# lukehinds/fastllm

Hardware: NVIDIA B200
Metric: decode_tokens_per_s (higher is better)
Workload: dtype bf16

## Files before the change

### fastllm_b200/csrc/decode_persistent.cuh

```cuda
#pragma once
#include "attn_decode.cuh"
#include "common.cuh"
#include "dense_ops.cuh"
#include "gemm_tc.cuh"
#include "gemv.cuh"
#include "mma.cuh"

namespace fl {

constexpr int kPkConsumerWarps = 8;
constexpr int kPkConsumers = kPkConsumerWarps * 32;
constexpr int kPkThreads = kPkConsumers + 32;
constexpr int kPkBlockRows = 16;
constexpr int kPkChunkCols = 1024;
constexpr int kPkStageBytes = kPkBlockRows * kPkChunkCols * 2;
constexpr int kPkMaxStages = 6;
constexpr int kPkMaxSlots = 96;
constexpr int kPkMaxNormK = 8192;

struct PkLayer {
    const uint16_t* wqkv;
    const float* bqkv;
    const uint16_t* wo;
    const uint16_t* wgu;
    const uint16_t* wdown;
    const float* ln1;
    const float* ln2;
};

struct PkArgs {
    const PkLayer* layers;
    int L;
    const uint16_t* embed;
    const uint16_t* lm_head;
    const float* final_norm;
    int H, I, V, nh, nkv, d, nqkv, max_pos;
    float eps, qscale;
    const float* rope_cos;
    const float* rope_sin;
    uint16_t* kpool;
    uint16_t* vpool;
    size_t layer_pool_elems;
    const int* page_table;
    StepState* state;
    float* resid;
    float* q;
    float* attn_out;
    uint16_t* xhl;
    float* act;
    float* logits;
    float* part_acc;
    float* part_ml;
    int* counters;
    int nsplit;
    float* amax_val;
    int* amax_idx;
    uint32_t* ids;
    uint32_t* next_ids;
    uint32_t* trace;
    int* trace_pos;
    unsigned int* gbar;
    int nsteps, feedback;
    int nstages;
    int xs_floats;
    int kcap;
    const CUtensorMap* tmaps;
    unsigned int* pool;
    int partial_rows;
    int tp, rank;
    float* peer_part[8];
    unsigned int* peer_flag[8];
    float* peer_amax[8];
    float* peer_logits[8];
    unsigned int ar_epoch0;
    int* comm_err;
    long long* dbg;
};

struct PkSplit {
    int s0, s1;
    int pool0, npool;
    int ncc;
};
constexpr int kPkStaticNum = 30;
constexpr int kPkPoolCap = 8;

__device__ __forceinline__ PkSplit pk_split(int N, int K, int cta, int ncta, bool dynamic) {
    PkSplit p;
    const int nblk = N / kPkBlockRows;
    p.ncc = (K + kPkChunkCols - 1) / kPkChunkCols;
    if (dynamic) {
        const int S = (int)((long long)nblk * kPkStaticNum / 32) / ncta;
        p.s0 = cta * S; p.s1 = p.s0 + S;
        p.pool0 = ncta * S; p.npool = nblk - p.pool0;
    } else {
        p.s0 = (int)((long long)nblk * cta / ncta); p.s1 = (int)((long long)nblk * (cta + 1) / ncta);
        p.pool0 = nblk; p.npool = 0;
    }
    return p;
}

constexpr int kPkMetaEnd = 1 << 30;

__device__ __forceinline__ void pk_named_sync() { asm volatile("bar.sync 1, %0;" ::"n"(kPkConsumers) : "memory"); }

__device__ __forceinline__ unsigned int ld_acquire_gpu(const unsigned int* p) {
    unsigned int v;
    asm volatile("ld.acquire.gpu.global.u32 %0, [%1];" : "=r"(v) : "l"(p) : "memory");
    return v;
}

__device__ __forceinline__ uint4 ldcg_u4(const void* p) {
    uint4 r;
    asm volatile("ld.global.cg.v4.u32 {%0, %1, %2, %3}, [%4];" : "=r"(r.x), "=r"(r.y), "=r"(r.z), "=r"(r.w) : "l"(p));
    return r;
}
// ... 8 lines not shown
    const PkLayer& lw = a.layers[g >> 2];
    switch (g & 3) {
        case 0: W = lw.wqkv; N = a.nqkv; K = a.H; break;
        case 1: W = lw.wo; N = a.H; K = a.nh * a.d; break;
        case 2: W = lw.wgu; N = 2 * a.I; K = a.H; break;
        default: W = lw.wdown; N = a.H; K = a.I; break;
    }
}

__device__ __forceinline__ void pk_grid_barrier(unsigned int* ctr, unsigned int& epoch, int tid) {
    pk_named_sync();
    epoch += 1;
    if (tid == 0) {
        asm volatile("red.release.gpu.global.add.u32 [%0], %1;" ::"l"(ctr), "r"(1u) : "memory");
        const unsigned int target = epoch * gridDim.x;
        while (ld_acquire_gpu(ctr) < target) { }
    }
    pk_named_sync();
}

__device__ __forceinline__ void st_release_sys(unsigned int* p, unsigned int v) {
    asm volatile("st.release.sys.global.u32 [%0], %1;" ::"l"(p), "r"(v) : "memory");
}
__device__ __forceinline__ unsigned int ld_acquire_sys(const unsigned int* p) {
    unsigned int v;
    asm volatile("ld.acquire.sys.global.u32 %0, [%1];" : "=r"(v) : "l"(p) : "memory");
    return v;
}
__device__ __forceinline__ void pk_wait_flag(const unsigned int* flag, unsigned int epoch, int* err) {
    const long long t0 = clock64();
    while ((int)(ld_acquire_sys(flag) - epoch) < 0) {
        if (clock64() - t0 > 4000000000LL) {
            *err = 1;
            break;
        }
    }
}

template <int D>
__global__ void __launch_bounds__(kPkThreads, 1) decode_persistent_kernel(const PkArgs a) {
    extern __shared__ __align__(1024) uint8_t smem[];
    uint8_t* ring = smem;
    float* xs = reinterpret_cast<float*>(smem + (size_t)a.nstages * kPkStageBytes);
    float* partial = xs + a.xs_floats;
    float* sc = partial + (size_t)a.partial_rows * kPkConsumerWarps;
    float* red = sc + kAttnMaxRep * kKvPage;
    float* alpha_s = red + 32;
    float* mrun = alpha_s + 8;
    float* lrun = mrun + 8;
    int* s_flag = reinterpret_cast<int*>(lrun + 8);
    __shared__ __align__(8) uint64_t full[kPkMaxStages];
    __shared__ __align__(8) uint64_t empty[kPkMaxStages];
    __shared__ __align__(8) uint64_t xbar;
    __shared__ int2 meta[kPkMaxStages];
    __shared__ int blk_rows[kPkMaxSlots];

    const int tid = threadIdx.x, lane = tid & 31, warp = tid >> 5;
    const int cta = blockIdx.x, ncta = gridDim.x;
    const int NS = a.nstages;
    const int nq = a.nh * a.d;

    if (tid == 0) {
        for (int s = 0; s < NS; ++s) {
            mbar_init(&full[s], 1);
            mbar_init(&empty[s], kPkConsumerWarps);
        }
        mbar_init(&xbar, 1);
        mbar_fence_init();
    }
    __syncthreads();

    if (warp == kPkConsumerWarps) {
        if (lane != 0) return;
        unsigned int c = 0;
        const uint64_t pol_first = l2_policy_evict_first();
        const bool dynamic = a.tp == 1 && a.pool != nullptr;
        for (int step = 0; step < a.nsteps; ++step) {
            for (int g = 0; g <= 4 * a.L; ++g) {
                const uint16_t* W;
                int N, K;
                pk_phase(a, g, W, N, K);
                const PkSplit sp = pk_split(N, K, cta, ncta, dynamic);
                const bool pdbg = a.dbg != nullptr && cta == 0 && g < 4 * a.L && (g >> 2) == a.L / 2;
                int pn = 0;
                auto fetch_block = [&](int blk) {
                    for (int cc = 0; cc < sp.ncc; ++cc) {
                        const int st = c % NS;
                        mbar_wait(&empty[st], ((c / NS) & 1) ^ 1);
                        ++c;
                        meta[st] = make_int2(blk * kPkBlockRows, cc | (cc == sp.ncc - 1 ? 1 << 16 : 0));
                        if (pdbg) {
                            long long t;
                            asm volatile("mov.u64 %0, %%globaltimer;" : "=l"(t));
                            if (pn < 8) a.dbg[660 + (g & 3) * 10 + pn] = t;
                            a.dbg[660 + (g & 3) * 10 + 8] = t;
                            a.dbg[660 + (g & 3) * 10 + 9] = ++pn;
                        }
                        mbar_expect_tx(&full[st], kPkStageBytes);
                        asm volatile(
                            "cp.async.bulk.tensor.3d.shared::cluster.global.mbarrier::complete_tx::bytes.L2::cache_hint [%0], [%1, {%2, %3, %4}], [%5], %6;" ::"r"(
                                smem_u32(ring + (size_t)st * kPkStageBytes)),
                            "l"(a.tmaps + g), "r"(0), "r"(blk * kPkBlockRows), "r"(cc * (kPkChunkCols / 64)), "r"(smem_u32(&full[st])), "l"(pol_first)
                            : "memory");
                    }
                };
                for (int blk = sp.s0; blk < sp.s1; ++blk) fetch_block(blk);
                for (int taken = 0; sp.npool > 0 && taken < kPkPoolCap; ++taken) {
                    const int t = (int)atomicAdd(a.pool + g, 1u);
                    if (t >= sp.npool) break;
                    fetch_block(sp.pool0 + t);
                }
                const int st = c % NS;
                mbar_wait(&empty[st], ((c / NS) & 1) ^ 1);
                meta[st] = make_int2(0, kPkMetaEnd);
                mbar_arrive(&full[st]);
                ++c;
            }
        }
        return;
    }
// ... 149 lines not shown
                    v[j] = make_float4(bf16lo(e.x), bf16hi(e.x), bf16lo(e.y), bf16hi(e.y));
                    if (resid_out) reinterpret_cast<float4*>(resid_out)[i] = v[j];
                } else {
                    v[j] = __ldcg(reinterpret_cast<const float4*>(src) + i);
                }
            }
        }
#pragma unroll
        for (int j = 0; j < NV; ++j) {
            ss = fmaf(v[j].x, v[j].x, ss); ss = fmaf(v[j].y, v[j].y, ss); ss = fmaf(v[j].z, v[j].z, ss); ss = fmaf(v[j].w, v[j].w, ss);
        }
        const float tot = block_sum(ss);
        const float m = sqrtf(tot / (float)K + a.eps);
#pragma unroll
        for (int j = 0; j < NV; ++j) {
            const int i = tid + j * kPkConsumers;
            const float4 x = v[j];
            if (i < K / 4) store_x4(i, make_float4(x.x / m * wv[j].x, x.y / m * wv[j].y, x.z / m * wv[j].z, x.w / m * wv[j].w));
        }
        zero_x_tail(K);
        pk_named_sync();
    };
    unsigned int xphase = 0;
    auto load_x_plain = [&](const uint16_t* hi, int K) {
        if (tid == 0) {
            asm volatile("fence.proxy.async;" ::: "memory");
            mbar_expect_tx(&xbar, (uint32_t)K * 4u);
            bulk_g2s(xh, hi, (uint32_t)K * 2u, &xbar);
            bulk_g2s(xl, hi + K, (uint32_t)K * 2u, &xbar);
        }
        zero_x_tail(K);
        mbar_wait(&xbar, xphase & 1u);
        xphase ^= 1u;
        pk_named_sync();
    };

    auto prefetch_vec = [&](const float* p, int n) {
        for (int i = tid * 32; i < n; i += kPkConsumers * 32) asm volatile("prefetch.global.L2 [%0];" ::"l"(p + i));
    };
    int dbg_i = 0;
    auto stamp = [&](int l) {
        if (a.dbg != nullptr && cta == 0 && tid == 0 && l == a.L / 2) {
            long long t;
            asm volatile("mov.u64 %0, %%globaltimer;" : "=l"(t));
            a.dbg[dbg_i] = t;
        }
        ++dbg_i;
    };
    const int n_rep = a.nh / a.nkv;
    constexpr int LPT = D / 8, TPW = 32 / LPT;
    const int grp = lane / LPT, gl = lane % LPT;
    int item0 = cta;
    asm volatile("" : "+r"(item0));

    for (int step = 0; step < a.nsteps; ++step) {
        const uint32_t tok_id = __ldcg(a.ids);
        const int rope_pos = min(__ldcg(&a.state->rope_pos), a.max_pos - 1);
        const int kv_base = __ldcg(&a.state->kv_base[0]);
        const int slot = kv_base;
        const int len = kv_base + 1;
        const int page_of_slot = __ldg(a.page_table + slot / kKvPage);

        for (int l = 0; l < a.L; ++l) {
            const PkLayer& lw = a.layers[l];
            uint16_t* kpool = a.kpool + (size_t)l * a.layer_pool_elems;
            uint16_t* vpool = a.vpool + (size_t)l * a.layer_pool_elems;

            prefetch_vec(lw.ln2, a.H);
            dbg_i = 0;
            dbg_layer = l;
            stamp(l);
            if (l == 0) {
                const int npages = (len + kKvPage - 1) / kKvPage;
                for (int i = tid * 32; i < npages; i += kPkConsumers * 32) asm volatile("prefetch.global.L1 [%0];" ::"l"(a.page_table + i));
            }
            if (l == 0)
                load_x_rmsnorm(nullptr, true, a.embed + (size_t)tok_id * a.H, lw.ln1, a.H, cta == 0 ? a.resid : nullptr);
            else
                load_x_rmsnorm(a.resid, false, nullptr, lw.ln1, a.H, nullptr);
            stamp(l);
            {
                const int nslots = consume(a.H);
                stamp(l);
                const int d = a.d, half = d >> 1;
                for (int e = tid; e < nslots * (kPkBlockRows / 2); e += kPkConsumers) {
                    const int ra = grow(2 * e);
                    float va = row_sum(2 * e), vb = row_sum(2 * e + 1);
                    if (lw.bqkv) { va += lw.bqkv[ra]; vb += lw.bqkv[ra + 1]; }
                    const int hh = ra / d, j = (ra % d) >> 1;
                    if (hh < a.nh + a.nkv) {
                        const float cs = a.rope_cos[(size_t)rope_pos * half + j], sn = a.rope_sin[(size_t)rope_pos * half + j];
                        const float o1 = va * cs - vb * sn, o2 = va * sn + vb * cs;
                        if (hh < a.nh) {
                            a.q[(size_t)hh * d + j] = o1;
                            a.q[(size_t)hh * d + j + half] = o2;
                        } else {
                            uint16_t* kp = kpool + (((size_t)page_of_slot * a.nkv + (hh - a.nh)) * kKvPage + slot % kKvPage) * d;
                            kp[j] = f32_to_bf16_rne(o1);
                            kp[j + half] = f32_to_bf16_rne(o2);
                        }
                    } else {
                        uint16_t* vp = vpool + (((size_t)page_of_slot * a.nkv + (hh - a.nh - a.nkv)) * kKvPage + slot % kKvPage) * d;
                        *reinterpret_cast<uint32_t*>(vp + 2 * j) = (uint32_t)f32_to_bf16_rne(va) | ((uint32_t)f32_to_bf16_rne(vb) << 16);
                    }
                }
            }
            stamp(l);
            pk_grid_barrier(a.gbar, epoch, tid);
            if (cta == 0 && tid == 0 && a.pool != nullptr) atomicExch(a.pool + (4 * l), 0u);
            stamp(l);

            {
                constexpr int HG = 4;
                constexpr int NG = kPkConsumerWarps * TPW;
                constexpr int BATCH = 4;
                const int npages = (len + kKvPage - 1) / kKvPage;
                const int per = (npages + a.nsplit - 1) / a.nsplit;
                float* gacc = xs;
                float* gml = xs + NG * HG * D;
                for (int item = item0; item < a.nkv * a.nsplit; item += ncta) {
                    const int kvh = item / a.nsplit, split = item % a.nsplit;
                    const int tok0 = split * per * kKvPage, tok1 = min(min((split + 1) * per, npages) * kKvPage, len);
                    const int gidx = warp * TPW + grp;
                    for (int h0 = 0; h0 < n_rep; h0 += HG) {
                        float qv[HG][8], acc[HG][8], mr[HG], lr[HG];
#pragma unroll
                        for (int h = 0; h < HG; ++h) {
                            mr[h] = -INFINITY;
                            lr[h] = 0.f;
#pragma unroll
                            for (int i = 0; i < 8; ++i) acc[h][i] = 0.f;
                            if (h0 + h < n_rep) {
                                const float4* qp = reinterpret_cast<const float4*>(a.q + (size_t)(kvh * n_rep + h0 + h) * D + gl * 8);
                                const float4 q0 = __ldcg(qp), q1 = __ldcg(qp + 1);
                                qv[h][0] = q0.x * a.qscale; qv[h][1] = q0.y * a.qscale; qv[h][2] = q0.z * a.qscale; qv[h][3] = q0.w * a.qscale;
                                qv[h][4] = q1.x * a.qscale; qv[h][5] = q1.y * a.qscale; qv[h][6] = q1.z * a.qscale; qv[h][7] = q1.w * a.qscale;
                            } else {
#pragma unroll
                                for (int i = 0; i < 8; ++i) qv[h][i] = 0.f;
                            }
                        }
                        for (int tb0 = tok0; tb0 < tok1; tb0 += NG * BATCH) {
                            const int tb = tb0 + gidx;
                            uint4 kw[BATCH], vw[BATCH];
#pragma unroll
                            for (int it = 0; it < BATCH; ++it) {
                                const int tk = tb + it * NG;
                                if (tk < tok1) {
                                    const size_t base = (((size_t)__ldg(a.page_table + tk / kKvPage) * a.nkv + kvh) * kKvPage + tk % kKvPage) * D + gl * 8;
                                    kw[it] = ldcg_u4(kpool + base);
                                    vw[it] = ldcg_u4(vpool + base);
                                } else {
                                    kw[it] = make_uint4(0u, 0u, 0u, 0u);
                                    vw[it] = kw[it];
                                }
                            }
#pragma unroll
                            for (int it = 0; it < BATCH; ++it) {
                                const bool valid = tb + it * NG < tok1;
                                const float kf[8] = {bf16lo(kw[it].x), bf16hi(kw[it].x), bf16lo(kw[it].y), bf16hi(kw[it].y),
                                                     bf16lo(kw[it].z), bf16hi(kw[it].z), bf16lo(kw[it].w), bf16hi(kw[it].w)};
                                const float vf[8] = {bf16lo(vw[it].x), bf16hi(vw[it].x), bf16lo(vw[it].y), bf16hi(vw[it].y),
                                                     bf16lo(vw[it].z), bf16hi(vw[it].z), bf16lo(vw[it].w), bf16hi(vw[it].w)};
#pragma unroll
                                for (int h = 0; h < HG; ++h) {
                                    float sv = kf[0] * qv[h][0];
#pragma unroll
                                    for (int i = 1; i < 8; ++i) sv = fmaf(kf[i], qv[h][i], sv);
#pragma unroll
                                    for (int o = LPT / 2; o > 0; o >>= 1) sv += __shfl_xor_sync(0xFFFFFFFFu, sv, o);
                                    if (valid) {
                                        const float m_new = fmaxf(mr[h], sv);
                                        const float al = expf(mr[h] - m_new), pr = expf(sv - m_new);
                                        lr[h] = lr[h] * al + pr;
                                        mr[h] = m_new;
#pragma unroll
                                        for (int i = 0; i < 8; ++i) acc[h][i] = fmaf(acc[h][i], al, pr * vf[i]);
                                    }
                                }
                            }
                        }
#pragma unroll
                        for (int h = 0; h < HG; ++h) {
                            float* dst = gacc + ((size_t)gidx * HG + h) * D + gl * 8;
#pragma unroll
                            for (int i = 0; i < 8; ++i) dst[i] = acc[h][i];
                            if (gl == 0) {
                                gml[(gidx * HG + h) * 2] = mr[h];
                                gml[(gidx * HG + h) * 2 + 1] = lr[h];
                            }
                        }
                        pk_named_sync();
                        for (int i = tid; i < HG * D; i += kPkConsumers) {
                            const int h = i / D, dd = i % D;
                            if (h0 + h < n_rep) {
                                float M = -INFINITY;
#pragma unroll
                                for (int g = 0; g < NG; ++g) M = fmaxf(M, gml[(g * HG + h) * 2]);
                                float num = 0.f, den = 0.f;
                                if (M != -INFINITY) {
#pragma unroll
                                    for (int g = 0; g < NG; ++g) {
                                        const float wg = expf(gml[(g * HG + h) * 2] - M);
                                        num = fmaf(wg, gacc[((size_t)g * HG + h) * D + dd], num);
                                        den = fmaf(wg, gml[(g * HG + h) * 2 + 1], den);
                                    }
                                }
                                const size_t pidx = (size_t)(kvh * n_rep + h0 + h) * a.nsplit + split;
                                a.part_acc[pidx * D + dd] = num;
                                if (dd == 0) {
                                    a.part_ml[pidx * 2] = M;
                                    a.part_ml[pidx * 2 + 1] = den;
                                }
                            }
                        }
                        pk_named_sync();
                    }
                    __threadfence();
                    pk_named_sync();
                    if (tid == 0) *s_flag = (atomicAdd(&a.counters[kvh], 1) == a.nsplit - 1);
                    pk_named_sync();
                    if (*s_flag) {
                        __threadfence();
                        float* cm = xs;
                        float* cden = cm + kAttnMaxRep * a.nsplit;
                        if (warp < n_rep) {
                            const int h = warp;
                            const size_t base = (size_t)(kvh * n_rep + h) * a.nsplit;
                            float mstar = -INFINITY;
                            for (int s = lane; s < a.nsplit; s += 32) mstar = fmaxf(mstar, __ldcg(a.part_ml + (base + s) * 2));
                            mstar = warp_max(mstar);
                            float den = 0.f;
                            for (int s = lane; s < a.nsplit; s += 32) {
                                const float ms = __ldcg(a.part_ml + (base + s) * 2);
                                const float w = (ms == -INFINITY) ? 0.f : expf(ms - mstar);
                                cm[h * a.nsplit + s] = w;
                                den = fmaf(w, __ldcg(a.part_ml + (base + s) * 2 + 1), den);
                            }
                            den = warp_sum(den);
                            if (lane == 0) cden[h] = den;
                        }
                        pk_named_sync();
                        constexpr int D4 = D / 4;
                        for (int i = tid; i < n_rep * D4; i += kPkConsumers) {
                            const int h = i / D4, c4 = i % D4;
                            const float4* src = reinterpret_cast<const float4*>(a.part_acc + (size_t)(kvh * n_rep + h) * a.nsplit * D) + c4;
                            float4 num = make_float4(0.f, 0.f, 0.f, 0.f);
#pragma unroll 8
                            for (int s = 0; s < a.nsplit; ++s) {
                                const float w = cm[h * a.nsplit + s];
                                if (w != 0.f) {
                                    const float4 v = __ldcg(src + (size_t)s * D4);
                                    num.x = fmaf(w, v.x, num.x); num.y = fmaf(w, v.y, num.y); num.z = fmaf(w, v.z, num.z); num.w = fmaf(w, v.w, num.w);
                                }
                            }
                            const float den = cden[h];
                            uint32_t h0, l0, h1, l1;
                            split2(num.x / den, num.y / den, h0, l0);
                            split2(num.z / den, num.w / den, h1, l1);
                            const size_t oi = (size_t)(kvh * n_rep + h) * D + c4 * 4;
                            *reinterpret_cast<uint2*>(a.xhl + oi) = make_uint2(h0, h1);
                            *reinterpret_cast<uint2*>(a.xhl + nq + oi) = make_uint2(l0, l1);
                        }
                        if (tid == 0) a.counters[kvh] = 0;
                    }
                    pk_named_sync();
                }
            }
            stamp(l);
            pk_grid_barrier(a.gbar, epoch, tid);
            stamp(l);

            prefetch_vec(l + 1 < a.L ? a.layers[l + 1].ln1 : a.final_norm, a.H);
            load_x_plain(a.xhl, nq);
            stamp(l);
            {
                const int nslots = consume(nq);
                stamp(l);
                if (a.tp > 1) {
                    allreduce_resid_add(nslots);
                } else {
                    for (int e = tid; e < nslots * (kPkBlockRows / 2); e += kPkConsumers) {
                        float2* p = reinterpret_cast<float2*>(a.resid + grow(2 * e));
                        float2 v = __ldcg(p);
                        v.x += row_sum(2 * e);
                        v.y += row_sum(2 * e + 1);
                        *p = v;
                    }
                }
            }
            stamp(l);
            pk_grid_barrier(a.gbar, epoch, tid);
            if (cta == 0 && tid == 0 && a.pool != nullptr) atomicExch(a.pool + (4 * l + 1), 0u);
            stamp(l);

            load_x_rmsnorm(a.resid, false, nullptr, lw.ln2, a.H, nullptr);
            stamp(l);
            {
                long long t0c = 0;
                if (a.dbg != nullptr && tid == 0 && l == a.L / 2) asm volatile("mov.u64 %0, %%globaltimer;" : "=l"(t0c));
                const int nslots = consume(a.H);
                if (a.dbg != nullptr && tid == 0 && l == a.L / 2) {
                    long long t1c;
                    unsigned int smid;
                    asm volatile("mov.u64 %0, %%globaltimer;" : "=l"(t1c));
                    asm volatile("mov.u32 %0, %%smid;" : "=r"(smid));
                    a.dbg[64 + cta * 4] = t0c; a.dbg[64 + cta * 4 + 1] = t1c; a.dbg[64 + cta * 4 + 2] = smid; a.dbg[64 + cta * 4 + 3] = nslots;
                }
                stamp(l);
                for (int e = tid; e < nslots * (kPkBlockRows / 2); e += kPkConsumers) {
                    const float g = row_sum(2 * e), u = row_sum(2 * e + 1);
                    const float av = g / (1.f + expf(-g)) * u;
                    uint16_t ah, al;
                    split_hi_lo(av, ah, al);
                    const int aj = grow(2 * e) >> 1;
                    a.xhl[2 * nq + aj] = ah;
                    a.xhl[2 * nq + a.I + aj] = al;
                }
            }
// ... 122 lines not shown
```

### fastllm_b200/csrc/fl_lib.cu

```cuda
#include <cmath>
#include <sstream>
#include <thread>

#include "attn_decode.cuh"
#include "attn_mma.cuh"
#include "comm.cuh"
#include "decode_persistent.cuh"
#include "dense_ops.cuh"
#include "gemm_tc.cuh"
#include "elementwise.cuh"
#include "gemv.cuh"
#include "model.cuh"
#include "sampler.hpp"
#include "synth.cuh"

namespace fl {

thread_local std::string g_last_error;
std::atomic<uint64_t> g_launches{0};
Profiler g_prof;
NcclApi g_nccl;
PeerComm g_peer;
static std::atomic<int> g_device{-1};

// ... 487 lines not shown
            tm.push_back(make_tmap_pk(w.layers[l].wdown, w.H, w.I));
        }
        tm.push_back(make_tmap_pk(w.lm_head, w.V, w.H));
        w.pk_tmaps.alloc(tm.size());
        FL_CUDA(cudaMemcpy(w.pk_tmaps.p, tm.data(), tm.size() * sizeof(CUtensorMap), cudaMemcpyHostToDevice));
    }
    w.finalized = true;
}

static void tp_allreduce_sum(LaunchCtx& lc, float* buf, size_t count) {
    FL_CHECK(g_nccl.comm != nullptr, FL_ERR_STATE, "tensor parallelism: fl_comm_init has not been called");
    g_nccl.check(g_nccl.AllReduce(buf, buf, count, ncclFloat32, ncclSum, g_nccl.comm, lc.stream), "ncclAllReduce");
    count_launch(lc);
}
static void tp_allgather(LaunchCtx& lc, const float* send, float* recv, size_t count) {
    FL_CHECK(g_nccl.comm != nullptr, FL_ERR_STATE, "tensor parallelism: fl_comm_init has not been called");
    g_nccl.check(g_nccl.AllGather(send, recv, count, ncclFloat32, g_nccl.comm, lc.stream), "ncclAllGather");
    count_launch(lc);
}
struct A2aSeg {
    const void* send;
    void* recv;
    size_t bytes;
    bool replicate;
};
static void ep_alltoall(LaunchCtx& lc, const A2aSeg* segs, int nseg) {
    FL_CHECK(g_nccl.comm != nullptr, FL_ERR_STATE, "expert parallelism: fl_comm_init has not been called");
    g_nccl.check(g_nccl.GroupStart(), "ncclGroupStart");
    for (int i = 0; i < nseg; ++i) {
        const A2aSeg& sg = segs[i];
        for (int p = 0; p < g_nccl.world; ++p) {
            const uint8_t* sp = (const uint8_t*)sg.send + (sg.replicate ? 0 : (size_t)p * sg.bytes);
            g_nccl.check(g_nccl.Send(sp, sg.bytes, ncclUint8, p, g_nccl.comm, lc.stream), "ncclSend");
            g_nccl.check(g_nccl.Recv((uint8_t*)sg.recv + (size_t)p * sg.bytes, sg.bytes, ncclUint8, p, g_nccl.comm, lc.stream), "ncclRecv");
        }
    }
    g_nccl.check(g_nccl.GroupEnd(), "ncclGroupEnd");
    count_launch(lc);
}

constexpr int kPassRows = 2;

static void plan_persistent(fl_cache& c) {
    const Weights& w = *c.w;
    PkPlan& p = c.pk;
    p.ok = false;
    if (env_flag("FL_NO_PERSISTENT")) return;
    if (w.tp > 1 && (!g_peer.ready || w.H > PeerComm::kMaxH || (size_t)w.Vfull > PeerComm::kMaxVocab || w.tp > PeerComm::kMaxTp)) return;
    if (w.cfg.arch == FL_ARCH_MIXTRAL) return;
    const int nq = w.nh * w.d;
    if (!(w.d == 64 || w.d == 128)) return;
    if (w.H < 2048 || nq < 256 || w.I < 256) return;
    if (w.pk_tmaps.p == nullptr || w.nqkv % 16 || w.H % 16 || (2 * w.I) % 16 || w.V % 16 || w.H > kPkMaxNormK) return;
    int kmax = (std::max(w.H, std::max(nq, w.I)) + kPkChunkCols - 1) / kPkChunkCols * kPkChunkCols;
    p.xs_floats = (int)align_up((size_t)std::max(std::max(kmax + 16, 8192 + 512), 8 * kNumSMs + 16), 4);
    int slots = 0;
    for (int N : {w.nqkv, w.H, 2 * w.I, w.V}) {
        const int nblk = N / kPkBlockRows;
        slots = std::max(slots, w.tp == 1 ? nblk / kNumSMs + kPkPoolCap : (nblk + kNumSMs - 1) / kNumSMs + 1);
    }
    if (slots > kPkMaxSlots) return;
    p.partial_rows = slots * kPkBlockRows;
    const size_t fixed = (size_t)p.xs_floats * 4 + (size_t)p.partial_rows * kPkConsumerWarps * 4 + (size_t)kAttnMaxRep * kKvPage * 4 + 64 * 4;
    const size_t avail = 232448 - 2048;
    if (fixed + 2 * (size_t)kPkStageBytes > avail) return;
    p.nstages = (int)std::min<size_t>(kPkMaxStages, (avail - fixed) / kPkStageBytes);
    p.smem = (size_t)p.nstages * kPkStageBytes + fixed;
    p.nsplit = std::max(1, std::min(c.pages_per_seq, kNumSMs / w.nkv));
    if (p.nsplit > c.nsplit) p.nsplit = c.nsplit;
    int coop = 0;
    FL_CUDA(cudaDeviceGetAttribute(&coop, cudaDevAttrCooperativeLaunch, w.device));
    if (!coop) return;
    c.gbar.alloc(1, true);
    p.ok = true;
}

static void launch_persistent(fl_cache& c, int nsteps, bool feedback) {
    const Weights& w = *c.w;
    PkArgs a{};
    a.layers = w.pk_layers.p; a.L = w.L; a.embed = w.embed; a.lm_head = w.lm_head; a.final_norm = w.final_norm;
    a.H = w.H; a.I = w.I; a.V = w.V; a.nh = w.nh; a.nkv = w.nkv; a.d = w.d; a.nqkv = w.nqkv; a.max_pos = w.max_pos;
    a.eps = w.cfg.norm_eps; a.qscale = (float)(1.0 / std::sqrt((double)w.d));
    a.rope_cos = w.rope_cos; a.rope_sin = w.rope_sin;
    a.kpool = c.kpool.p; a.vpool = c.vpool.p; a.layer_pool_elems = c.layer_pool_elems; a.page_table = c.page_table.p;
    a.state = c.state.p; a.resid = c.resid.p; a.q = c.q.p; a.attn_out = c.attn_out.p; a.act = c.act.p; a.logits = c.logits.p;
    a.part_acc = c.part_acc.p; a.part_ml = c.part_ml.p; a.counters = c.counters.p; a.nsplit = c.pk.nsplit;
    a.amax_val = c.amax_val.p; a.amax_idx = c.amax_idx.p; a.ids = c.ids.p; a.next_ids = c.next_ids.p;
    a.trace = feedback ? c.trace.p : nullptr; a.trace_pos = c.trace_pos.p; a.gbar = c.gbar.p;
    a.nsteps = nsteps; a.feedback = feedback ? 1 : 0; a.nstages = c.pk.nstages; a.xs_floats = c.pk.xs_floats;
    a.partial_rows = c.pk.partial_rows;
    if (c.pk_xhl.p == nullptr) c.pk_xhl.alloc(2 * ((size_t)w.nh * w.d + w.I) + 64, true);
    a.xhl = c.pk_xhl.p;
    a.kcap = (std::max(w.H, std::max(w.nh * w.d, w.I)) + kPkChunkCols - 1) / kPkChunkCols * kPkChunkCols;
    a.tmaps = w.pk_tmaps.p;
    if (c.pk_pool.p == nullptr) c.pk_pool.alloc(4 * (size_t)w.L + 1, true);
    a.pool = c.pk_pool.p;
    a.tp = w.tp; a.rank = w.rank;
    if (w.tp > 1) {
        for (int r = 0; r < w.tp; ++r) {
            uint8_t* base = (uint8_t*)g_peer.peer[r];
            a.peer_part[r] = (float*)(base + PeerComm::kPartOff);
            a.peer_flag[r] = (unsigned int*)(base + PeerComm::kFlagOff);
            a.peer_amax[r] = (float*)(base + PeerComm::kAmaxOff);
            a.peer_logits[r] = (float*)(base + PeerComm::kLogitsOff);
        }
        a.comm_err = (int*)((uint8_t*)g_peer.local + PeerComm::kErrOff);
        a.ar_epoch0 = g_peer.ar_epoch;
        g_peer.ar_epoch += (unsigned int)nsteps * (2u * (unsigned int)w.L + 1u);
    }
    static long long* dbg_buf = nullptr;
    const bool dbg = env_flag("FL_PK_DEBUG");
    if (dbg && !dbg_buf) {
        FL_CUDA(cudaMalloc(&dbg_buf, (64 + 4 * kNumSMs + 64) * sizeof(long long)));
        FL_CUDA(cudaMemset(dbg_buf, 0, (64 + 4 * kNumSMs + 64) * sizeof(long long)));
    }
    a.dbg = dbg ? dbg_buf : nullptr;
    FL_CUDA(cudaMemsetAsync(c.gbar.p, 0, sizeof(unsigned int), c.stream));
    FL_CUDA(cudaMemsetAsync(c.pk_pool.p, 0, (4 * (size_t)w.L + 1) * sizeof(unsigned int), c.stream));
    LaunchCtx lc{c.stream, false};
    lc.cooperative = true;
    const uint64_t bytes = (uint64_t)nsteps * (w.streamed_bytes + (uint64_t)c.kv_len * w.L * w.nkv * w.d * 2 * 2);
    with_head_dim(w.d, [&](auto D) {
        if constexpr (D == 64 || D == 128)
            launch(lc, "decode_persistent", bytes, decode_persistent_kernel<D>, dim3(kNumSMs), dim3(kPkThreads), c.pk.smem, a);
    });
    if (w.tp > 1)
        FL_CUDA(cudaMemcpyAsync(c.logits.p, (uint8_t*)g_peer.local + PeerComm::kLogitsOff, (size_t)w.Vfull * 4, cudaMemcpyDeviceToDevice, c.stream));
    if (dbg) {
        static const char* names[] = {"P1 x(rmsnorm)", "P1 consume qkv", "P1 epilogue", "P1 grid barrier", "P2 attention", "P2 grid barrier",
                                      "P3 x", "P3 consume o", "P3 epilogue", "P3 grid barrier", "P4 x(rmsnorm)", "P4 consume gate/up",
                                      "P4 epilogue", "P4 grid barrier", "P5 x", "P5 consume down", "P5 epilogue", "P5 grid barrier"};
        long long h[40];
        FL_CUDA(cudaStreamSynchronize(c.stream));
        FL_CUDA(cudaMemcpy(h, dbg_buf, sizeof(h), cudaMemcpyDeviceToHost));
        fprintf(stderr, "[FL_PK_DEBUG] warp 0 of CTA 0, clocks waiting for weights / chunks per phase: qkv %lld/%lld o %lld/%lld gateup %lld/%lld down %lld/%lld\n",
                h[32] / 1000, h[32] % 1000, h[33] / 1000, h[33] % 1000, h[34] / 1000, h[34] % 1000, h[35] / 1000, h[35] % 1000);
        fprintf(stderr, "[FL_PK_DEBUG] layer %d, CTA 0 phase times (us):", w.L / 2);
        for (int i = 0; i < 18; ++i) fprintf(stderr, " %s=%.2f;", names[i], (h[i + 1] - h[i]) / 1000.0);
        fprintf(stderr, " layer total=%.2f\n", (h[18] - h[0]) / 1000.0);
        {
            long long pr[40];
            FL_CUDA(cudaMemcpy(pr, dbg_buf + 660, sizeof(pr), cudaMemcpyDeviceToHost));
// ... 1174 lines not shown
```

### fastllm_b200/csrc/model.cuh

```cuda
#pragma once
#include <map>
#include <memory>
#include <set>
#include <string>
#include <vector>

#include "../../include/fastllm_b200.h"
#include "bert_model.cuh"
#include "decode_persistent.cuh"
#include "gemv.cuh"
#include "runtime.cuh"

namespace fl {

struct LayerW {
    uint16_t* wqkv = nullptr;
    float* bqkv = nullptr;
    uint16_t* wo = nullptr;
    uint16_t* wgu = nullptr;
    uint16_t* wdown = nullptr;
    float* ln1 = nullptr;
    float* ln2 = nullptr;
    CUtensorMap tm_wqkv, tm_wo, tm_wgu, tm_wdown;
    float* wgate = nullptr;
    std::vector<uint16_t*> ewgu, ewdown;
    std::vector<CUtensorMap> tm_ewgu, tm_ewdown;
    CUtensorMap tm_ewgu_all, tm_ewdown_all;
};

struct Weights {
    fl_config cfg{};
    int H = 0, I = 0, V = 0, L = 0, nh = 0, nkv = 0, d = 0, max_pos = 0;
    int nqkv = 0;
    int tp = 1, rank = 0;
    int q_head0 = 0, q_real = 0, kv_head0 = 0;
    int E = 0, top_k = 0;
    int ep = 1, E_local = 0;
    bool ep_dp = false;
    int Vfull = 0;
    int device = 0;
    DevBuf<uint8_t> slab;
    uint16_t* embed = nullptr;
    uint16_t* lm_head = nullptr;
    float* final_norm = nullptr;
    std::vector<LayerW> layers;
    DevBuf<PkLayer> pk_layers;
    DevBuf<CUtensorMap> pk_tmaps;
    float* rope_cos = nullptr;
    float* rope_sin = nullptr;
    std::set<std::string> have;
    bool lm_head_loaded = false;
    bool finalized = false;
    uint64_t streamed_bytes = 0;
    CUtensorMap tm_head;
    bool dense_ok = false;
    std::mutex mu;
};

struct PkPlan {
    bool ok = false;
    int nstages = 0, xs_floats = 0, partial_rows = 0, nsplit = 1;
    size_t smem = 0;
};

struct DenseWs {
    size_t rows = 0;
    DevBuf<uint16_t> xhi, xlo;
    DevBuf<float> y;
    DevBuf<float> resid, q;
    DevBuf<float> tp_buf;
    DevBuf<uint16_t> xhi2, xlo2;
    DevBuf<uint16_t> vt;
    size_t vt_pages_cap = 0;
    CUtensorMap tm_vt{};
    DevBuf<float> sk_acc, sk_ml;
    DevBuf<float> moe_out, route_w;
    DevBuf<int> route_sel;
    DevBuf<float> route_margin;
    int route_rows = 0;
    DevBuf<uint16_t> gx_hi, gx_lo;
    DevBuf<int> grp_cnt, grp_pos;
    DevBuf<uint16_t> g_xhi, g_xlo;
    DevBuf<float> g_route;
    DevBuf<float> comb;
    DevBuf<int> counters;
};

struct GraphKey {
    int b;
    int loop;
    bool operator<(const GraphKey& o) const { return b != o.b ? b < o.b : loop < o.loop; }
};
struct GraphEntry {
    cudaGraphExec_t exec = nullptr;
    uint64_t kernels = 0;
};

}

struct fl_model {
    std::shared_ptr<fl::Weights> w;
    std::shared_ptr<fl::BertModel> bert;
};

struct fl_cache {
    std::shared_ptr<fl::Weights> w;
    cudaStream_t stream = nullptr;
    int max_batch = 0, max_seq = 0, pages_per_seq = 0, nsplit = 1;
    int kv_len = 0;
    bool slots_used = false;
    std::vector<int> slot_len;
    fl::DevBuf<int> slot_tab;
    fl::PinnedBuf<int> h_slot_tab;
    fl::DevBuf<uint32_t> sample_out;
// ... 28 lines not shown
```

Baseline: 330.6.

## Prefetch KV pages into shared memory via bulk async copy before attention

During the QKV projection phase, one consumer thread issues bulk global-to-shared copies of this CTA's KV-cache pages into the xs scratch region, tracked by a new mbarrier. The attention loop then reads K/V from shared memory, overlapping KV fetch latency with the QKV epilogue and grid barrier. The plan sizes stage_pages to fit leftover shared memory, and attention is restricted to one item per CTA. The final combine is also restructured to use acq_rel atomics and cache ml values in shared memory. This adds shared memory pressure, which may reduce pipeline stages, and a one-item-per-CTA assumption.

```diff
diff --git a/fastllm_b200/csrc/decode_persistent.cuh b/fastllm_b200/csrc/decode_persistent.cuh
--- a/fastllm_b200/csrc/decode_persistent.cuh
+++ b/fastllm_b200/csrc/decode_persistent.cuh
@@ -17,6 +17,8 @@
 constexpr int kPkMaxStages = 6;
 constexpr int kPkMaxSlots = 96;
 constexpr int kPkMaxNormK = 8192;
+constexpr int kPkAttnHeads = 4;
+constexpr size_t pk_attn_scratch_floats(int d) { return (size_t)kPkConsumerWarps * (32 / (d / 8)) * kPkAttnHeads * (d + 2); }
 
 struct PkLayer {
     const uint16_t* wqkv;
@@ -62,6 +64,7 @@
     unsigned int* gbar;
     int nsteps, feedback;
     int nstages;
+    int stage_pages;
     int xs_floats;
     int kcap;
     const CUtensorMap* tmaps;
@@ -176,6 +179,7 @@
     __shared__ __align__(8) uint64_t full[kPkMaxStages];
     __shared__ __align__(8) uint64_t empty[kPkMaxStages];
     __shared__ __align__(8) uint64_t xbar;
+    __shared__ __align__(8) uint64_t kvbar;
     __shared__ int2 meta[kPkMaxStages];
     __shared__ int blk_rows[kPkMaxSlots];
 
@@ -190,6 +194,7 @@
             mbar_init(&empty[s], kPkConsumerWarps);
         }
         mbar_init(&xbar, 1);
+        mbar_init(&kvbar, 1);
         mbar_fence_init();
     }
     __syncthreads();
@@ -445,6 +450,21 @@
     const int grp = lane / LPT, gl = lane % LPT;
     int item0 = cta;
     asm volatile("" : "+r"(item0));
+    const bool has_item = item0 < a.nkv * a.nsplit;
+    struct PkItem { int kvh, split, tok0, tok1; };
+    auto item_of = [&](int len) {
+        int item = item0;
+        asm volatile("" : "+r"(item));
+        const int npages = (len + kKvPage - 1) / kKvPage, per = (npages + a.nsplit - 1) / a.nsplit;
+        PkItem it;
+        it.kvh = item / a.nsplit;
+        it.split = item % a.nsplit;
+        it.tok0 = it.split * per * kKvPage;
+        it.tok1 = min(min((it.split + 1) * per, npages) * kKvPage, len);
+        return it;
+    };
+    auto stage_k = [&]() { return reinterpret_cast<uint16_t*>(xs); };
+    auto stage_v = [&]() { return reinterpret_cast<uint16_t*>(xs) + (size_t)a.stage_pages * kKvPage * D; };
 
     for (int step = 0; step < a.nsteps; ++step) {
         const uint32_t tok_id = __ldcg(a.ids);
@@ -475,6 +495,18 @@
             {
                 const int nslots = consume(a.H);
                 stamp(l);
+                if (has_item && tid == kPkConsumers - 1) {
+                    const PkItem it = item_of(len);
+                    const int ts1 = max(it.tok0, min(min(it.tok0 + a.stage_pages * kKvPage, it.tok1), slot));
+                    asm volatile("fence.proxy.async;" ::: "memory");
+                    mbar_expect_tx(&kvbar, (uint32_t)(ts1 - it.tok0) * D * 4u);
+                    for (int t = it.tok0; t < ts1; t += kKvPage) {
+                        const size_t src = ((size_t)__ldg(a.page_table + t / kKvPage) * a.nkv + it.kvh) * kKvPage * D;
+                        const uint32_t bytes = (uint32_t)min(kKvPage, ts1 - t) * D * 2u;
+                        bulk_g2s(stage_k() + (size_t)(t - it.tok0) * D, kpool + src, bytes, &kvbar);
+                        bulk_g2s(stage_v() + (size_t)(t - it.tok0) * D, vpool + src, bytes, &kvbar);
+                    }
+                }
                 const int d = a.d, half = d >> 1;
                 for (int e = tid; e < nslots * (kPkBlockRows / 2); e += kPkConsumers) {
                     const int ra = grow(2 * e);
@@ -503,161 +535,176 @@
             if (cta == 0 && tid == 0 && a.pool != nullptr) atomicExch(a.pool + (4 * l), 0u);
             stamp(l);
 
-            {
-                constexpr int HG = 4;
+            if (has_item) {
+                constexpr int HG = kPkAttnHeads;
                 constexpr int NG = kPkConsumerWarps * TPW;
                 constexpr int BATCH = 4;
-                const int npages = (len + kKvPage - 1) / kKvPage;
-                const int per = (npages + a.nsplit - 1) / a.nsplit;
-                float* gacc = xs;
-                float* gml = xs + NG * HG * D;
-                for (int item = item0; item < a.nkv * a.nsplit; item += ncta) {
-                    const int kvh = item / a.nsplit, split = item % a.nsplit;
-                    const int tok0 = split * per * kKvPage, tok1 = min(min((split + 1) * per, npages) * kKvPage, len);
-                    const int gidx = warp * TPW + grp;
-                    for (int h0 = 0; h0 < n_rep; h0 += HG) {
-                        float qv[HG][8], acc[HG][8], mr[HG], lr[HG];
-#pragma unroll
-                        for (int h = 0; h < HG; ++h) {
-                            mr[h] = -INFINITY;
-                            lr[h] = 0.f;
-#pragma unroll
-                            for (int i = 0; i < 8; ++i) acc[h][i] = 0.f;
-                            if (h0 + h < n_rep) {
-                                const float4* qp = reinterpret_cast<const float4*>(a.q + (size_t)(kvh * n_rep + h0 + h) * D + gl * 8);
-                                const float4 q0 = __ldcg(qp), q1 = __ldcg(qp + 1);
-                                qv[h][0] = q0.x * a.qscale; qv[h][1] = q0.y * a.qscale; qv[h][2] = q0.z * a.qscale; qv[h][3] = q0.w * a.qscale;
-                                qv[h][4] = q1.x * a.qscale; qv[h][5] = q1.y * a.qscale; qv[h][6] = q1.z * a.qscale; qv[h][7] = q1.w * a.qscale;
+                const PkItem it = item_of(len);
+                const int kvh = it.kvh, split = it.split, tok0 = it.tok0, tok1 = it.tok1;
+                const int tst = min(tok0 + a.stage_pages * kKvPage, tok1);
+                float* gacc = n_rep <= HG ? xs : reinterpret_cast<float*>(stage_v() + (size_t)a.stage_pages * kKvPage * D);
+                float* gml = gacc + NG * HG * D;
+                const int gidx = warp * TPW + grp;
+                for (int h0 = 0; h0 < n_rep; h0 += HG) {
+                    float qv[HG][8], acc[HG][8], mr[HG], lr[HG];
+#pragma unroll
+                    for (int h = 0; h < HG; ++h) {
+                        mr[h] = -INFINITY;
+                        lr[h] = 0.f;
+#pragma unroll
+                        for (int i = 0; i < 8; ++i) acc[h][i] = 0.f;
+                        if (h0 + h < n_rep) {
+                            const float4* qp = reinterpret_cast<const float4*>(a.q + (size_t)(kvh * n_rep + h0 + h) * D + gl * 8);
+                            const float4 q0 = __ldcg(qp), q1 = __ldcg(qp + 1);
+                            qv[h][0] = q0.x * a.qscale; qv[h][1] = q0.y * a.qscale; qv[h][2] = q0.z * a.qscale; qv[h][3] = q0.w * a.qscale;
+                            qv[h][4] = q1.x * a.qscale; qv[h][5] = q1.y * a.qscale; qv[h][6] = q1.z * a.qscale; qv[h][7] = q1.w * a.qscale;
+                        } else {
+#pragma unroll
+                            for (int i = 0; i < 8; ++i) qv[h][i] = 0.f;
+                        }
+                    }
+                    if (h0 == 0) {
+                        if (slot >= tok0 && slot < tst && (slot - tok0) % NG == gidx) {
+                            const size_t base = (((size_t)page_of_slot * a.nkv + kvh) * kKvPage + slot % kKvPage) * D + gl * 8;
+                            *reinterpret_cast<uint4*>(stage_k() + (size_t)(slot - tok0) * D + gl * 8) = ldcg_u4(kpool + base);
+                            *reinterpret_cast<uint4*>(stage_v() + (size_t)(slot - tok0) * D + gl * 8) = ldcg_u4(vpool + base);
+                        }
+                        mbar_wait(&kvbar, (uint32_t)(step * a.L + l) & 1u);
+                    }
+                    for (int tb0 = tok0; tb0 < tok1; tb0 += NG * BATCH) {
+                        const int tb = tb0 + gidx;
+                        uint4 kw[BATCH], vw[BATCH];
+#pragma unroll
+                        for (int it = 0; it < BATCH; ++it) {
+                            const int tk = tb + it * NG;
+                            if (tk < tst) {
+                                kw[it] = *reinterpret_cast<const uint4*>(stage_k() + (size_t)(tk - tok0) * D + gl * 8);
+                                vw[it] = *reinterpret_cast<const uint4*>(stage_v() + (size_t)(tk - tok0) * D + gl * 8);
+                            } else if (tk < tok1) {
+                                const size_t base = (((size_t)__ldg(a.page_table + tk / kKvPage) * a.nkv + kvh) * kKvPage + tk % kKvPage) * D + gl * 8;
+                                kw[it] = ldcg_u4(kpool + base);
+                                vw[it] = ldcg_u4(vpool + base);
                             } else {
-#pragma unroll
-                                for (int i = 0; i < 8; ++i) qv[h][i] = 0.f;
+                                kw[it] = make_uint4(0u, 0u, 0u, 0u);
+                                vw[it] = kw[it];
                             }
                         }
-                        for (int tb0 = tok0; tb0 < tok1; tb0 += NG * BATCH) {
-                            const int tb = tb0 + gidx;
-                            uint4 kw[BATCH], vw[BATCH];
-#pragma unroll
-                            for (int it = 0; it < BATCH; ++it) {
-                                const int tk = tb + it * NG;
-                                if (tk < tok1) {
-                                    const size_t base = (((size_t)__ldg(a.page_table + tk / kKvPage) * a.nkv + kvh) * kKvPage + tk % kKvPage) * D + gl * 8;
-                                    kw[it] = ldcg_u4(kpool + base);
-                                    vw[it] = ldcg_u4(vpool + base);
-                                } else {
-                                    kw[it] = make_uint4(0u, 0u, 0u, 0u);
-                                    vw[it] = kw[it];
+#pragma unroll
+                        for (int it = 0; it < BATCH; ++it) {
+                            const bool valid = tb + it * NG < tok1;
+                            const float kf[8] = {bf16lo(kw[it].x), bf16hi(kw[it].x), bf16lo(kw[it].y), bf16hi(kw[it].y),
+                                                 bf16lo(kw[it].z), bf16hi(kw[it].z), bf16lo(kw[it].w), bf16hi(kw[it].w)};
+                            const float vf[8] = {bf16lo(vw[it].x), bf16hi(vw[it].x), bf16lo(vw[it].y), bf16hi(vw[it].y),
+                                                 bf16lo(vw[it].z), bf16hi(vw[it].z), bf16lo(vw[it].w), bf16hi(vw[it].w)};
+#pragma unroll
+                            for (int h = 0; h < HG; ++h) {
+                                float sv = kf[0] * qv[h][0];
+#pragma unroll
+                                for (int i = 1; i < 8; ++i) sv = fmaf(kf[i], qv[h][i], sv);
+#pragma unroll
+                                for (int o = LPT / 2; o > 0; o >>= 1) sv += __shfl_xor_sync(0xFFFFFFFFu, sv, o);
+                                if (valid) {
+                                    const float m_new = fmaxf(mr[h], sv);
+                                    const float al = expf(mr[h] - m_new), pr = expf(sv - m_new);
+                                    lr[h] = lr[h] * al + pr;
+                                    mr[h] = m_new;
+#pragma unroll
+                                    for (int i = 0; i < 8; ++i) acc[h][i] = fmaf(acc[h][i], al, pr * vf[i]);
                                 }
                             }
-#pragma unroll
-                            for (int it = 0; it < BATCH; ++it) {
-                                const bool valid = tb + it * NG < tok1;
-                                const float kf[8] = {bf16lo(kw[it].x), bf16hi(kw[it].x), bf16lo(kw[it].y), bf16hi(kw[it].y),
-                                                     bf16lo(kw[it].z), bf16hi(kw[it].z), bf16lo(kw[it].w), bf16hi(kw[it].w)};
-                                const float vf[8] = {bf16lo(vw[it].x), bf16hi(vw[it].x), bf16lo(vw[it].y), bf16hi(vw[it].y),
-                                                     bf16lo(vw[it].z), bf16hi(vw[it].z), bf16lo(vw[it].w), bf16hi(vw[it].w)};
-#pragma unroll
-                                for (int h = 0; h < HG; ++h) {
-                                    float sv = kf[0] * qv[h][0];
-#pragma unroll
-                                    for (int i = 1; i < 8; ++i) sv = fmaf(kf[i], qv[h][i], sv);
-#pragma unroll
-                                    for (int o = LPT / 2; o > 0; o >>= 1) sv += __shfl_xor_sync(0xFFFFFFFFu, sv, o);
-                                    if (valid) {
-                                        const float m_new = fmaxf(mr[h], sv);
-                                        const float al = expf(mr[h] - m_new), pr = expf(sv - m_new);
-                                        lr[h] = lr[h] * al + pr;
-                                        mr[h] = m_new;
-#pragma unroll
-                                        for (int i = 0; i < 8; ++i) acc[h][i] = fmaf(acc[h][i], al, pr * vf[i]);
-                                    }
+                        }
+                    }
+                    if (n_rep <= HG) pk_named_sync();
+#pragma unroll
+                    for (int h = 0; h < HG; ++h) {
+                        float* dst = gacc + ((size_t)gidx * HG + h) * D + gl * 8;
+#pragma unroll
+                        for (int i = 0; i < 8; ++i) dst[i] = acc[h][i];
+                        if (gl == 0) {
+                            gml[(gidx * HG + h) * 2] = mr[h];
+                            gml[(gidx * HG + h) * 2 + 1] = lr[h];
+                        }
+                    }
+                    pk_named_sync();
+                    for (int i = tid; i < HG * D; i += kPkConsumers) {
+                        const int h = i / D, dd = i % D;
+                        if (h0 + h < n_rep) {
+                            float M = -INFINITY;
+#pragma unroll
+                            for (int g = 0; g < NG; ++g) M = fmaxf(M, gml[(g * HG + h) * 2]);
+                            float num = 0.f, den = 0.f;
+                            if (M != -INFINITY) {
+#pragma unroll
+                                for (int g = 0; g < NG; ++g) {
+                                    const float wg = expf(gml[(g * HG + h) * 2] - M);
+                                    num = fmaf(wg, gacc[((size_t)g * HG + h) * D + dd], num);
+                                    den = fmaf(wg, gml[(g * HG + h) * 2 + 1], den);
                                 }
                             }
-                        }
-#pragma unroll
-                        for (int h = 0; h < HG; ++h) {
-                            float* dst = gacc + ((size_t)gidx * HG + h) * D + gl * 8;
-#pragma unroll
-                            for (int i = 0; i < 8; ++i) dst[i] = acc[h][i];
-                            if (gl == 0) {
-                                gml[(gidx * HG + h) * 2] = mr[h];
-                                gml[(gidx * HG + h) * 2 + 1] = lr[h];
+                            const size_t pidx = (size_t)(kvh * n_rep + h0 + h) * a.nsplit + split;
+                            a.part_acc[pidx * D + dd] = num;
+                            if (dd == 0) {
+                                a.part_ml[pidx * 2] = M;
+                                a.part_ml[pidx * 2 + 1] = den;
                             }
                         }
-                        pk_named_sync();
-                        for (int i = tid; i < HG * D; i += kPkConsumers) {
-                            const int h = i / D, dd = i % D;
-                            if (h0 + h < n_rep) {
-                                float M = -INFINITY;
-#pragma unroll
-                                for (int g = 0; g < NG; ++g) M = fmaxf(M, gml[(g * HG + h) * 2]);
-                                float num = 0.f, den = 0.f;
-                                if (M != -INFINITY) {
-#pragma unroll
-                                    for (int g = 0; g < NG; ++g) {
-                                        const float wg = expf(gml[(g * HG + h) * 2] - M);
-                                        num = fmaf(wg, gacc[((size_t)g * HG + h) * D + dd], num);
-                                        den = fmaf(wg, gml[(g * HG + h) * 2 + 1], den);
-                                    }
-                                }
-                                const size_t pidx = (size_t)(kvh * n_rep + h0 + h) * a.nsplit + split;
-                                a.part_acc[pidx * D + dd] = num;
-                                if (dd == 0) {
-                                    a.part_ml[pidx * 2] = M;
-                                    a.part_ml[pidx * 2 + 1] = den;
-                                }
+                    }
+                    pk_named_sync();
+                }
+                if (tid == 0) {
+                    int prev;
+                    asm volatile("atom.acq_rel.gpu.global.add.s32 %0, [%1], 1;" : "=r"(prev) : "l"(a.counters + kvh) : "memory");
+                    *s_flag = prev == a.nsplit - 1;
+                }
+                pk_named_sync();
+                if (*s_flag) {
+                    constexpr int D4 = D / 4;
+                    float* cm = gacc;
+                    float* cden = cm + kAttnMaxRep * a.nsplit;
+                    float* cl = cden + kAttnMaxRep;
+                    if (warp < n_rep) {
+                        const int h = warp;
+                        const float2* ml = reinterpret_cast<const float2*>(a.part_ml) + (size_t)(kvh * n_rep + h) * a.nsplit;
+                        float mstar = -INFINITY;
+                        for (int s = lane; s < a.nsplit; s += 32) {
+                            const float2 v = __ldcg(ml + s);
+                            cm[h * a.nsplit + s] = v.x;
+                            cl[h * a.nsplit + s] = v.y;
+                            mstar = fmaxf(mstar, v.x);
+                        }
+                        mstar = warp_max(mstar);
+                        float den = 0.f;
+                        for (int s = lane; s < a.nsplit; s += 32) {
+                            const float ms = cm[h * a.nsplit + s];
+                            const float w = (ms == -INFINITY) ? 0.f : expf(ms - mstar);
+                            cm[h * a.nsplit + s] = w;
+                            den = fmaf(w, cl[h * a.nsplit + s], den);
+                        }
+                        den = warp_sum(den);
+                        if (lane == 0) cden[h] = den;
+                    }
+                    pk_named_sync();
+                    if (tid < n_rep * D4) {
+                        const int hm = tid / D4, c4 = tid % D4;
+                        const float4* src = reinterpret_cast<const float4*>(a.part_acc + (size_t)(kvh * n_rep + hm) * a.nsplit * D) + c4;
+                        float4 num = make_float4(0.f, 0.f, 0.f, 0.f);
+#pragma unroll 8
+                        for (int s = 0; s < a.nsplit; ++s) {
+                            const float w = cm[hm * a.nsplit + s];
+                            if (w != 0.f) {
+                                const float4 v = __ldcg(src + (size_t)s * D4);
+                                num.x = fmaf(w, v.x, num.x); num.y = fmaf(w, v.y, num.y); num.z = fmaf(w, v.z, num.z); num.w = fmaf(w, v.w, num.w);
                             }
                         }
-                        pk_named_sync();
-                    }
-                    __threadfence();
-                    pk_named_sync();
-                    if (tid == 0) *s_flag = (atomicAdd(&a.counters[kvh], 1) == a.nsplit - 1);
-                    pk_named_sync();
-                    if (*s_flag) {
-                        __threadfence();
-                        float* cm = xs;
-                        float* cden = cm + kAttnMaxRep * a.nsplit;
-                        if (warp < n_rep) {
-                            const int h = warp;
-                            const size_t base = (size_t)(kvh * n_rep + h) * a.nsplit;
-                            float mstar = -INFINITY;
-                            for (int s = lane; s < a.nsplit; s += 32) mstar = fmaxf(mstar, __ldcg(a.part_ml + (base + s) * 2));
-                            mstar = warp_max(mstar);
-                            float den = 0.f;
-                            for (int s = lane; s < a.nsplit; s += 32) {
-                                const float ms = __ldcg(a.part_ml + (base + s) * 2);
-                                const float w = (ms == -INFINITY) ? 0.f : expf(ms - mstar);
-                                cm[h * a.nsplit + s] = w;
-                                den = fmaf(w, __ldcg(a.part_ml + (base + s) * 2 + 1), den);
-                            }
-                            den = warp_sum(den);
-                            if (lane == 0) cden[h] = den;
-                        }
-                        pk_named_sync();
-                        constexpr int D4 = D / 4;
-                        for (int i = tid; i < n_rep * D4; i += kPkConsumers) {
-                            const int h = i / D4, c4 = i % D4;
-                            const float4* src = reinterpret_cast<const float4*>(a.part_acc + (size_t)(kvh * n_rep + h) * a.nsplit * D) + c4;
-                            float4 num = make_float4(0.f, 0.f, 0.f, 0.f);
-#pragma unroll 8
-                            for (int s = 0; s < a.nsplit; ++s) {
-                                const float w = cm[h * a.nsplit + s];
-                                if (w != 0.f) {
-                                    const float4 v = __ldcg(src + (size_t)s * D4);
-                                    num.x = fmaf(w, v.x, num.x); num.y = fmaf(w, v.y, num.y); num.z = fmaf(w, v.z, num.z); num.w = fmaf(w, v.w, num.w);
-                                }
-                            }
-                            const float den = cden[h];
-                            uint32_t h0, l0, h1, l1;
-                            split2(num.x / den, num.y / den, h0, l0);
-                            split2(num.z / den, num.w / den, h1, l1);
-                            const size_t oi = (size_t)(kvh * n_rep + h) * D + c4 * 4;
-                            *reinterpret_cast<uint2*>(a.xhl + oi) = make_uint2(h0, h1);
-                            *reinterpret_cast<uint2*>(a.xhl + nq + oi) = make_uint2(l0, l1);
-                        }
-                        if (tid == 0) a.counters[kvh] = 0;
-                    }
-                    pk_named_sync();
+                        const float den = cden[hm];
+                        uint32_t h0, l0, h1, l1;
+                        split2(num.x / den, num.y / den, h0, l0);
+                        split2(num.z / den, num.w / den, h1, l1);
+                        const size_t oi = (size_t)(kvh * n_rep + hm) * D + c4 * 4;
+                        *reinterpret_cast<uint2*>(a.xhl + oi) = make_uint2(h0, h1);
+                        *reinterpret_cast<uint2*>(a.xhl + nq + oi) = make_uint2(l0, l1);
+                    }
+                    if (tid == 0) a.counters[kvh] = 0;
                 }
             }
             stamp(l);
diff --git a/fastllm_b200/csrc/fl_lib.cu b/fastllm_b200/csrc/fl_lib.cu
--- a/fastllm_b200/csrc/fl_lib.cu
+++ b/fastllm_b200/csrc/fl_lib.cu
@@ -563,8 +563,16 @@
     if (!(w.d == 64 || w.d == 128)) return;
     if (w.H < 2048 || nq < 256 || w.I < 256) return;
     if (w.pk_tmaps.p == nullptr || w.nqkv % 16 || w.H % 16 || (2 * w.I) % 16 || w.V % 16 || w.H > kPkMaxNormK) return;
-    int kmax = (std::max(w.H, std::max(nq, w.I)) + kPkChunkCols - 1) / kPkChunkCols * kPkChunkCols;
-    p.xs_floats = (int)align_up((size_t)std::max(std::max(kmax + 16, 8192 + 512), 8 * kNumSMs + 16), 4);
+    p.nsplit = std::max(1, std::min(c.pages_per_seq, kNumSMs / w.nkv));
+    if (p.nsplit > c.nsplit) p.nsplit = c.nsplit;
+    const size_t kmax = (std::max(w.H, std::max(nq, w.I)) + kPkChunkCols - 1) / kPkChunkCols * kPkChunkCols;
+    const size_t page_floats = (size_t)2 * kKvPage * w.d / 2;
+    const size_t scratch = pk_attn_scratch_floats(w.d);
+    const bool one_pass = w.nh / w.nkv <= kPkAttnHeads;
+    auto xs_floats = [&](int pages) {
+        const size_t att = one_pass ? std::max((size_t)pages * page_floats, scratch) : (size_t)pages * page_floats + scratch;
+        return align_up(std::max(kmax + 16, att), 4);
+    };
     int slots = 0;
     for (int N : {w.nqkv, w.H, 2 * w.I, w.V}) {
         const int nblk = N / kPkBlockRows;
@@ -572,13 +580,15 @@
     }
     if (slots > kPkMaxSlots) return;
     p.partial_rows = slots * kPkBlockRows;
-    const size_t fixed = (size_t)p.xs_floats * 4 + (size_t)p.partial_rows * kPkConsumerWarps * 4 + (size_t)kAttnMaxRep * kKvPage * 4 + 64 * 4;
+    const size_t other = (size_t)p.partial_rows * kPkConsumerWarps * 4 + (size_t)kAttnMaxRep * kKvPage * 4 + 64 * 4;
     const size_t avail = 232448 - 2048;
-    if (fixed + 2 * (size_t)kPkStageBytes > avail) return;
-    p.nstages = (int)std::min<size_t>(kPkMaxStages, (avail - fixed) / kPkStageBytes);
+    if (xs_floats(0) * 4 + other + 2 * (size_t)kPkStageBytes > avail) return;
+    p.nstages = (int)std::min<size_t>(kPkMaxStages, (avail - xs_floats(0) * 4 - other) / kPkStageBytes);
+    p.stage_pages = (c.pages_per_seq + p.nsplit - 1) / p.nsplit;
+    while (p.stage_pages > 0 && xs_floats(p.stage_pages) * 4 + other + (size_t)p.nstages * kPkStageBytes > avail) --p.stage_pages;
+    p.xs_floats = (int)xs_floats(p.stage_pages);
+    const size_t fixed = (size_t)p.xs_floats * 4 + other;
     p.smem = (size_t)p.nstages * kPkStageBytes + fixed;
-    p.nsplit = std::max(1, std::min(c.pages_per_seq, kNumSMs / w.nkv));
-    if (p.nsplit > c.nsplit) p.nsplit = c.nsplit;
     int coop = 0;
     FL_CUDA(cudaDeviceGetAttribute(&coop, cudaDevAttrCooperativeLaunch, w.device));
     if (!coop) return;
@@ -598,7 +608,7 @@
     a.part_acc = c.part_acc.p; a.part_ml = c.part_ml.p; a.counters = c.counters.p; a.nsplit = c.pk.nsplit;
     a.amax_val = c.amax_val.p; a.amax_idx = c.amax_idx.p; a.ids = c.ids.p; a.next_ids = c.next_ids.p;
     a.trace = feedback ? c.trace.p : nullptr; a.trace_pos = c.trace_pos.p; a.gbar = c.gbar.p;
-    a.nsteps = nsteps; a.feedback = feedback ? 1 : 0; a.nstages = c.pk.nstages; a.xs_floats = c.pk.xs_floats;
+    a.nsteps = nsteps; a.feedback = feedback ? 1 : 0; a.nstages = c.pk.nstages; a.stage_pages = c.pk.stage_pages; a.xs_floats = c.pk.xs_floats;
     a.partial_rows = c.pk.partial_rows;
     if (c.pk_xhl.p == nullptr) c.pk_xhl.alloc(2 * ((size_t)w.nh * w.d + w.I) + 64, true);
     a.xhl = c.pk_xhl.p;
diff --git a/fastllm_b200/csrc/model.cuh b/fastllm_b200/csrc/model.cuh
--- a/fastllm_b200/csrc/model.cuh
+++ b/fastllm_b200/csrc/model.cuh
@@ -59,7 +59,7 @@
 
 struct PkPlan {
     bool ok = false;
-    int nstages = 0, xs_floats = 0, partial_rows = 0, nsplit = 1;
+    int nstages = 0, xs_floats = 0, partial_rows = 0, nsplit = 1, stage_pages = 0;
     size_t smem = 0;
 };
 
```

New measurement: 334.7, median of 6. 1.2% higher.
